# lh3/bwa

Hardware: NVIDIA H100
Metric: reads_per_sec (higher is better)
Workload: dtype int32

## Files before the change

bwa_b200/csrc/cuda/bwag_api.cu:

```cuda
#include <stdio.h>
#include <stdlib.h>
#include <string.h>
#include <stdarg.h>
#include <pthread.h>
#include <time.h>
#include <math.h>
#include <sched.h>
#include "bwag_dev.cuh"
#include "bwag_kernels.h"

struct BlobHeader {
	u64 magic, primary, seq_len, bwt_size, n_sa, l_pac;
	u64 L2[5];
	u64 sa_shift;
	u64 off_bwt, off_sa, off_pac, total;
	u64 sb[BWAG_MAX_SB][4];
};
#define BLOB_MAGIC 0x3142574142323030ull
#define ALIGN256(x) (((x) + 255) & ~(size_t)255)

static __thread char g_err[512];
extern "C" const char *bwag_last_error(void) { return g_err[0] ? g_err : "no error"; }
static int set_err(const char *fmt, ...)
{
	va_list ap;
	va_start(ap, fmt);
	vsnprintf(g_err, sizeof(g_err), fmt, ap);
	va_end(ap);
	return 1;
}
int bwag_set_error(const char *msg) { return set_err("%s", msg); }
#define CK(call) do { cudaError_t e_ = (call); if (e_ != cudaSuccess) return set_err("%s failed at %s:%d: %s", #call, __FILE__, __LINE__, cudaGetErrorString(e_)); } while (0)
#define CKP(call) do { cudaError_t e_ = (call); if (e_ != cudaSuccess) { set_err("%s failed at %s:%d: %s", #call, __FILE__, __LINE__, cudaGetErrorString(e_)); return 0; } } while (0)

struct Counters {
	int next_read, next_task, max_rlen, next_read3;
	u64 next_seed;
	u64 n_intv, n_seeds;
	u64 occ_touches, sa_touches, ext_cells, glb_cells;
	u64 n_cig, n_md;
	u32 flags, n_pre;
	u64 t_dregs, t_tasks, t_max_z, t_text, t_complex;
	int t_max_lq, t_max_rl;
	int n_many;
	int n_big;
	u32 n_swtasks;
	u64 fm_total[3];
	int aln_next;
	u32 aln_redo, aln_flags;
	u64 aln_pool, aln_total;
	u64 se_total, se_run, se_cells;
	int se_next, se_past;
	u64 pm_total;
};

struct DevBuf { void *p; size_t cap; };
static int buf_reserve(DevBuf *b, size_t bytes)
{
	if (bytes <= b->cap) return 0;
	if (b->p) cudaFree(b->p);
	b->p = 0; b->cap = 0;
	size_t want = bytes + bytes / 4 + 256;
	CK(cudaMalloc(&b->p, want));
	b->cap = want;
	return 0;
}
struct HostBuf { void *p; size_t cap; };
static int hbuf_reserve(HostBuf *b, size_t bytes)
{
	if (bytes <= b->cap) return 0;
	if (b->p) cudaFreeHost(b->p);
	b->p = 0; b->cap = 0;
	size_t want = bytes + bytes / 4 + 256;
	CK(cudaMallocHost(&b->p, want));
	b->cap = want;
	return 0;
}

struct bwag_ctx {
	int device, own_blob, n_sm;
	int imported;
	size_t map_bytes[3];
	void *blob;
	DevIndex ix;
	u64 *dense_sa;
	ulonglong2 *ktab;
	int baseline;
	cudaStream_t stream;
	cudaEvent_t ev0, ev1, ev_wait;
	Counters *d_cnt, *h_cnt;
	bwag_stats_t st;
	int sa_intv_disk;
	DevBuf s_k1, s_k1f, s_n3, s_eh, s_rseq, s_qseq, s_z, s_wcig, s_wmd, s_pack, s_zl;
	int grid_k1, grid_k1f, grid_k2, grid_k4, grid_k5;
	int k3s_blocks;
#define N_SPARE 12
	struct bwag_batch *spare[N_SPARE];
	pthread_mutex_t mu;
	struct bwag_ctx *parent;
	void *d_tail; TailCtg tctg; const double *d_logtab; int have_ctg;
	void *d_ambs; int n_holes, have_ambs;
};

struct bwag_batch {
	bwag_ctx_t *ctx;
	bwag_ctx_t lc;
	int lc_ready;
	int n;
	i64 total_bases;
	int max_len;
	const i64 *h_off;
	DevBuf d_codes, d_off;
	DevBuf d_intv_beg, d_intv_n, d_intv, d_seed_beg, d_rbeg;
	HostBuf h_intv_beg, h_intv_n, h_intv, h_seed_beg, h_rbeg;
	DevBuf d_chain_off, d_chains, d_seeds, d_regs, d_nregs;
	DevBuf d_chain_beg, d_chain_cnt, d_reg_base, d_chain_rid, d_chain_frac, d_cregs, d_creg_beg, d_ctg;
	DevBuf s_bt, s_sn, s_ch, s_order, s_idx, s_keys;
	HostBuf h_regs, h_nregs, h_cregs, h_creg_beg, h_tmp;
	i64 n_intv, n_seeds;
	int seeded;
	DevBuf d_tasks, d_res, d_cig, d_md;
	HostBuf h_res, h_cig, h_md;
	DevBuf d_dregs, d_dreg_beg, d_dreg_n, d_task_beg, d_cflag, d_pe_is, d_rec, d_text, d_ptab;
	DevBuf d_swtasks, d_swres, d_swpool, d_swscratch; HostBuf h_swres;
	DevBuf d_hsp, d_flt_nchn; HostBuf h_hsp;
	DevBuf d_k3big;
	DevBuf d_pre_n, d_pre_score, d_pre_cig;
	DevBuf d_sel;
	HostBuf h_pe_is, h_cflag, h_rec, h_text, h_ptab;
	DevBuf d_fm_lbeg, d_fm_lines, d_fm_nrow, d_fm_rbeg, d_fm_rows, d_fm_tlen, d_fm_tbeg, d_fm_text, d_fm_toff;
	HostBuf h_fm_text, h_fm_off;
	DevBuf d_aln_md, d_aln_n, d_aln_beg, d_aln_pool, d_aln_redo[2], d_aln_off, d_aln_out, d_aln_arena;
	HostBuf h_aln_n, h_aln_off, h_aln_out;
	DevBuf d_se_reads, d_se_multi, d_se_bc, d_se_rows, d_se_pos, d_se_mpos, d_se_flags, d_se_tasks, d_se_mtask, d_se_cig, d_se_ncig, d_se_scratch, d_se_tlen, d_se_tbeg, d_se_rec, d_se_text, d_se_nm;
	HostBuf h_se_tasks, h_se_mtask, h_se_rec, h_se_text;
	DevBuf d_pe_rlen, d_pe_reads, d_pe_gtasks, d_pe_gres, d_pe_gcig, d_pe_pool;
	HostBuf h_pe_pos, h_pe_gres, h_pe_gcig;
	DevBuf d_pm_qual, d_pm_hasq, d_pm_names, d_pm_noff, d_pm_q, d_pm_code, d_pm_ovl, d_pm_tlen, d_pm_tbeg, d_pm_text, d_pm_cnt;
	HostBuf h_pm_text, h_pm_cnt;
	int tail_ready;
	int regs_on_device;
};

static void batch_free(bwag_batch_t *b);
static void free_dev(DevBuf *b) { if (b->p) cudaFree(b->p); b->p = 0; b->cap = 0; }
static void free_host(HostBuf *b) { if (b->p) cudaFreeHost(b->p); b->p = 0; b->cap = 0; }

#ifndef BWAG_L2_FETCH_DEFAULT
#define BWAG_L2_FETCH_DEFAULT 0
#endif
#define K1_SMEM_MAX (200 * 1024)
#ifndef K1_COMPACT_DEFAULT
#define K1_COMPACT_DEFAULT 1
#endif
#ifdef BWAG_CUSIM
#define BWAG_KTAB_MAX_AUTO 5
#else
#define BWAG_KTAB_MAX_AUTO 14
#endif
#define K4_SMEM_MAX (96 * 1024)
#define K4L_SMEM_MAX (200 * 1024)
#define SEEDSW_MAXLEN 200

#ifdef BWAG_CUSIM
unsigned long long bwag_cusim_sector_loads, bwag_cusim_list_acc[5];
#endif


extern "C" size_t bwag_blob_bytes(const bwt_t *bwt, int64_t l_pac)
{
	return ALIGN256(sizeof(BlobHeader)) + ALIGN256((size_t)bwt->bwt_size * 4 + 64) + ALIGN256((size_t)bwt->n_sa * 8 + 32) + ALIGN256((size_t)l_pac / 4 + 1 + 64);
}

extern "C" int bwag_blob_fill(int device, void *d_blob, const bwt_t *bwt, int64_t l_pac, const uint8_t *pac)
{
	BlobHeader h;
	if (device >= 0) CK(cudaSetDevice(device));
	memset(&h, 0, sizeof(h));
	h.magic = BLOB_MAGIC; h.primary = bwt->primary; h.seq_len = bwt->seq_len; h.bwt_size = bwt->bwt_size; h.n_sa = bwt->n_sa; h.l_pac = (u64)l_pac;
	for (int i = 0; i < 5; ++i) h.L2[i] = bwt->L2[i];
	{
		int s = 0;
		while ((1 << s) < bwt->sa_intv) ++s;
		if ((1 << s) != bwt->sa_intv) return set_err("suffix-array interval %d is not a power of two", bwt->sa_intv);
		h.sa_shift = (u64)s;
	}
	if (bwt->seq_len >= (u64)BWAG_MAX_SB << BWAG_SB_SHIFT) return set_err("index too large: %llu BWT symbols", (unsigned long long)bwt->seq_len);
	for (u64 s = 0; s << BWAG_SB_SHIFT < bwt->seq_len; ++s) {
		const u64 *cnt = (const u64 *)(bwt->bwt + ((s << BWAG_SB_SHIFT) >> 7) * 16);
		for (int k = 0; k < 4; ++k) h.sb[s][k] = cnt[k];
	}
	h.off_bwt = ALIGN256(sizeof(BlobHeader));
	h.off_sa = h.off_bwt + ALIGN256((size_t)bwt->bwt_size * 4 + 64);
	h.off_pac = h.off_sa + ALIGN256((size_t)bwt->n_sa * 8 + 32);
// ... 1669 lines not shown
		CK(cudaEventRecord(c->ev0, c->stream));
		BWAG_LAUNCH(k_chain_emit, (n + K3_THREADS - 1) / K3_THREADS, K3_THREADS, 0, c->stream, k);
		CK(cudaGetLastError());
		CK(cudaEventRecord(c->ev1, c->stream));
		if (fetch_counters(c)) return 1;
		c->st.ms_chain += elapsed_at(c, "chain", __LINE__); ++c->st.n_launch;
	}

	const int cap_q = (b->max_len + 3) & ~3;
	const int cap_r = (c->h_cnt->max_rlen + 16 + 15) & ~15;
	CK(cudaMemsetAsync(&c->d_cnt->next_read, 0, sizeof(int), c->stream));
	int grid = c->grid_k4;
	{
		i64 need = ((i64)n + (K4_THREADS / 32) - 1) / (K4_THREADS / 32);
		if (grid > need) grid = (int)(need > 0 ? need : 1);
	}
	ExtArgs a;
	memset(&a, 0, sizeof(a));
	a.codes = (const uint8_t *)b->d_codes.p; a.off = (const i64 *)b->d_off.p; a.n_reads = n; a.par = *par;
	a.chain_beg = (const i64 *)b->d_chain_beg.p; a.chain_cnt = (const int *)b->d_chain_cnt.p; a.reg_base = (const i64 *)b->d_reg_base.p;
	a.chains = (const bwag_xchain_t *)b->d_chains.p; a.seeds = (const bwag_xseed_t *)b->d_seeds.p;
	a.regs = (bwag_xreg_t *)b->d_regs.p; a.n_regs = (int32_t *)b->d_nregs.p;
	a.cap_q = cap_q; a.cap_r = cap_r; a.min_seed = cp->min_seed_len;
	a.next_read = &c->d_cnt->next_read; a.cells = &c->d_cnt->ext_cells; a.flags = &c->d_cnt->flags;
	CK(cudaEventRecord(c->ev0, c->stream));
	if (launch_extend(c, a, n, c->h_cnt->n_many)) return 1;
	CK(cudaEventRecord(c->ev1, c->stream));
	if (!out) {
		if (fetch_counters(c)) return 1;
		c->st.ms_extend += elapsed_at(c, "extend", __LINE__); ++c->st.n_launch;
		if (c->h_cnt->flags & 2u) return set_err("extension: a read or reference window exceeded the scratch capacity");
		c->st.ext_cells += c->h_cnt->ext_cells;
		b->regs_on_device = 1;
		return 0;
	}
	RegCompactArgs rc;
	rc.n_reads = n; rc.n_regs = (const int *)b->d_nregs.p; rc.regs = (const bwag_xreg_t *)b->d_regs.p; rc.reg_base = (const i64 *)b->d_reg_base.p;
	rc.chain_beg = (const i64 *)b->d_chain_beg.p; rc.chain_rid = (const int *)b->d_chain_rid.p; rc.chain_frac = (const float *)b->d_chain_frac.p;
	rc.out_beg = (i64 *)b->d_creg_beg.p; rc.total = &c->d_cnt->n_cig;
	if (buf_reserve(&b->d_cregs, sizeof(bwag_creg_t) * (size_t)(ns + 1))) return 1;
	rc.out = (bwag_creg_t *)b->d_cregs.p;
	BWAG_LAUNCH(k_regs_compact, (n + 127) / 128, 128, 0, c->stream, rc);
	CK(cudaGetLastError());
	if (fetch_counters(c)) return 1;
	c->st.ms_extend += elapsed_at(c, "extend", __LINE__); c->st.n_launch += 2;
	if (c->h_cnt->flags & 2u) return set_err("extension: a read or reference window exceeded the scratch capacity");
	c->st.ext_cells += c->h_cnt->ext_cells;
	const i64 n_regs = (i64)c->h_cnt->n_cig;
	if (hbuf_reserve(&b->h_cregs, sizeof(bwag_creg_t) * (size_t)(n_regs + 1)) || hbuf_reserve(&b->h_creg_beg, 8 * (size_t)(n + 1)) || hbuf_reserve(&b->h_nregs, 4 * (size_t)(n + 1))) return 1;
	CK(cudaEventRecord(c->ev0, c->stream));
	if (n_regs) D2H(c, b->h_cregs.p, b->d_cregs.p, sizeof(bwag_creg_t) * (size_t)n_regs);
	D2H(c, b->h_creg_beg.p, b->d_creg_beg.p, 8 * (size_t)n);
	D2H(c, b->h_nregs.p, b->d_nregs.p, 4 * (size_t)n);
	CK(cudaEventRecord(c->ev1, c->stream));
	CK(stream_wait(c));
	c->st.ms_d2h += elapsed_at(c, "d2h", __LINE__);
	out->n_regs = (const int32_t *)b->h_nregs.p; out->reg_beg = (const int64_t *)b->h_creg_beg.p; out->regs = (const bwag_creg_t *)b->h_cregs.p;
	return 0;
}

extern "C" int bwag_fetch_cregs(bwag_batch_t *b, int n_sel, const int32_t *sel, bwag_cregs_t *out)
{
	bwag_ctx_t *c = &b->lc;
	CK(cudaSetDevice(c->device));
	if (!b->regs_on_device) return set_err("bwag_fetch_cregs needs a preceding bwag_chain_extend(..., NULL) on the same batch");
	out->n_regs = 0; out->reg_beg = 0; out->regs = 0;
	if (n_sel <= 0) return 0;
	const i64 ns = b->n_seeds;
	if (buf_reserve(&b->d_cregs, sizeof(bwag_creg_t) * (size_t)(ns + 1)) || buf_reserve(&b->d_creg_beg, 8 * (size_t)(b->n + 1)) || buf_reserve(&b->d_sel, 8 * (size_t)(n_sel + 1))) return 1;
	if (reset_counters(c)) return 1;
	H2D(c, b->d_sel.p, sel, 4 * (size_t)n_sel);
	RegCompactArgs rc;
	rc.n_reads = b->n; rc.n_regs = (const int *)b->d_nregs.p; rc.regs = (const bwag_xreg_t *)b->d_regs.p; rc.reg_base = (const i64 *)b->d_reg_base.p;
	rc.chain_beg = (const i64 *)b->d_chain_beg.p; rc.chain_rid = (const int *)b->d_chain_rid.p; rc.chain_frac = (const float *)b->d_chain_frac.p;
	rc.out_beg = (i64 *)b->d_creg_beg.p; rc.total = &c->d_cnt->n_cig; rc.out = (bwag_creg_t *)b->d_cregs.p;
	int *d_out_n = (int *)b->d_sel.p + n_sel;
	BWAG_LAUNCH(k_regs_compact_sel, (n_sel + 127) / 128, 128, 0, c->stream, rc, (const int *)b->d_sel.p, n_sel, d_out_n);
	CK(cudaGetLastError());
	if (fetch_counters(c)) return 1;
	++c->st.n_launch;
	const i64 n_regs = (i64)c->h_cnt->n_cig;
	if (hbuf_reserve(&b->h_cregs, sizeof(bwag_creg_t) * (size_t)(n_regs + 1)) || hbuf_reserve(&b->h_creg_beg, 8 * (size_t)(n_sel + 1)) || hbuf_reserve(&b->h_nregs, 4 * (size_t)(n_sel + 1))) return 1;
	CK(cudaEventRecord(c->ev0, c->stream));
	if (n_regs) D2H(c, b->h_cregs.p, b->d_cregs.p, sizeof(bwag_creg_t) * (size_t)n_regs);
	D2H(c, b->h_creg_beg.p, b->d_creg_beg.p, 8 * (size_t)n_sel);
	D2H(c, b->h_nregs.p, d_out_n, 4 * (size_t)n_sel);
	CK(cudaEventRecord(c->ev1, c->stream));
	CK(stream_wait(c));
	c->st.ms_d2h += elapsed_at(c, "d2h", __LINE__);
	out->n_regs = (const int32_t *)b->h_nregs.p; out->reg_beg = (const int64_t *)b->h_creg_beg.p; out->regs = (const bwag_creg_t *)b->h_cregs.p;
	return 0;
}


static int run_global(bwag_batch_t *b, const bwag_sw_par_t *par, int n_tasks, int cap_q, int cap_r, i64 cap_z, i64 n_aln, i64 *nc_out, i64 *nm_out)
{
	bwag_ctx_t *c = &b->lc;
	cap_q = (cap_q + 3) & ~3; cap_r = (cap_r + 15) & ~15; cap_z = (cap_z + 15) & ~(i64)15;
	if (cap_q < 4) cap_q = 4;
	if (cap_r < 16) cap_r = 16;
	if (cap_z < 64) cap_z = 64;
	const int cap_wcig = cap_q + cap_r + 4, cap_wmd = 3 * cap_r + cap_q + 16;
	int grid = c->grid_k5;
	const int k5_zsm = getenv("BWA_B200_K5_ZSM") ? atoi(getenv("BWA_B200_K5_ZSM")) & ~15 : 6144;
	const int k5_per_warp = ((8 * (cap_q + 2) + cap_r + cap_q + 2 + 15) & ~15) + k5_zsm;
	const size_t k5_smem = (size_t)k5_per_warp * (K5_THREADS / 32);
	int k5_sm = k5_smem <= K4_SMEM_MAX && !(getenv("BWA_B200_K5_SM") && atoi(getenv("BWA_B200_K5_SM")) == 0);
	const int k5_fast = !c->baseline && !(getenv("BWA_B200_K5_FAST") && atoi(getenv("BWA_B200_K5_FAST")) == 0);
#ifndef BWAG_CUSIM
	if (k5_sm) { int nb = 0; CK(cudaOccupancyMaxActiveBlocksPerMultiprocessor(&nb, k5_fast ? k_global_sm_fast : k_global_sm, K5_THREADS, k5_smem)); if (nb < 2) k5_sm = 0; else grid = c->n_sm * nb; }
#endif
	{
		i64 need = ((i64)n_tasks + (K5_THREADS / 32) - 1) / (K5_THREADS / 32);
		if (grid > need) grid = (int)(need > 0 ? need : 1);
		i64 max_warps = ((i64)8 << 30) / cap_z;
		if (max_warps < K5_THREADS / 32) max_warps = K5_THREADS / 32;
		if ((i64)grid * (K5_THREADS / 32) > max_warps) grid = (int)(max_warps / (K5_THREADS / 32));
	}
	const size_t n_warps = (size_t)grid * (K5_THREADS / 32);
	if (buf_reserve(&c->s_eh, n_warps * 2 * (size_t)(cap_q + 2) * 4) || buf_reserve(&c->s_rseq, n_warps * (size_t)cap_r) ||
	    buf_reserve(&c->s_qseq, n_warps * (size_t)(cap_q + 2)) || buf_reserve(&c->s_z, n_warps * (size_t)cap_z) ||
	    buf_reserve(&c->s_wcig, n_warps * (size_t)cap_wcig * 4) || buf_reserve(&c->s_wmd, n_warps * (size_t)cap_wmd)) return 1;
	if (buf_reserve(&b->d_res, sizeof(bwag_gres_t) * (size_t)n_tasks)) return 1;
	int k5_lane = !c->baseline && cap_q <= K5L_QWORDS * 4 && n_tasks >= 64 && getenv("BWA_B200_K5_LANE") && atoi(getenv("BWA_B200_K5_LANE")) != 0;
	const size_t k5l_smem = (size_t)K5L_RING * K5L_THREADS * 8 + (size_t)K5L_QWORDS * K5L_THREADS * 4;
	const i64 k5l_cap_z = (i64)(K5L_RING - 1) * (cap_r < 1024 ? cap_r : 1024);
	int k5l_grid = 0;
	if (k5_lane) {
#ifndef BWAG_CUSIM
		int nb = 0;
		CK(cudaFuncSetAttribute(k_global_lane, cudaFuncAttributeMaxDynamicSharedMemorySize, (int)k5l_smem));
		CK(cudaOccupancyMaxActiveBlocksPerMultiprocessor(&nb, k_global_lane, K5L_THREADS, k5l_smem));
		k5l_grid = c->n_sm * (nb > 0 ? nb : 1);
#else
		k5l_grid = 2;
#endif
		const i64 need = ((i64)n_tasks + K5L_THREADS - 1) / K5L_THREADS;
		if (k5l_grid > need) k5l_grid = (int)need;
		if (buf_reserve(&b->d_pre_n, 4 * (size_t)n_tasks) || buf_reserve(&b->d_pre_score, 4 * (size_t)n_tasks) || buf_reserve(&b->d_pre_cig, 4 * (size_t)K5L_MAXCIG * (size_t)n_tasks) ||
		    buf_reserve(&c->s_zl, (size_t)k5l_cap_z * (size_t)k5l_grid * K5L_THREADS)) return 1;
	}
	i64 cap_cig = n_aln * 6 + 1024, cap_md = n_aln * 24 + 4096;
	for (int attempt = 0;; ++attempt) {
		if (buf_reserve(&b->d_cig, 4 * (size_t)cap_cig) || buf_reserve(&b->d_md, (size_t)cap_md)) return 1;
		GlbArgs a;
		memset(&a, 0, sizeof(a));
		a.codes = (const uint8_t *)b->d_codes.p; a.off = (const i64 *)b->d_off.p; a.par = *par;
		a.tasks = (const bwag_gtask_t *)b->d_tasks.p; a.n_tasks = n_tasks;
		a.res = (bwag_gres_t *)b->d_res.p; a.cigar = (u32 *)b->d_cig.p; a.md = (char *)b->d_md.p;
		a.cap_cig = cap_cig; a.cap_md = cap_md; a.n_cig = &c->d_cnt->n_cig; a.n_md = &c->d_cnt->n_md;
		a.w_cig = (u32 *)c->s_wcig.p; a.w_md = (char *)c->s_wmd.p; a.cap_wcig = cap_wcig; a.cap_wmd = cap_wmd;
		a.eh = (int *)c->s_eh.p; a.rseq = (uint8_t *)c->s_rseq.p; a.qseq = (uint8_t *)c->s_qseq.p; a.z = (uint8_t *)c->s_z.p;
		a.cap_q = cap_q; a.cap_r = cap_r; a.cap_z = cap_z;
		a.next_task = &c->d_cnt->next_task; a.cells = &c->d_cnt->glb_cells; a.flags = &c->d_cnt->flags;
		if (reset_counters(c)) return 1;
		CK(cudaEventRecord(c->ev0, c->stream));
		if (k5_lane) {
			GlbLaneArgs la;
			memset(&la, 0, sizeof(la));
			la.codes = a.codes; la.off = a.off; la.par = *par; la.tasks = a.tasks; la.n_tasks = n_tasks;
			la.pre_n = (int *)b->d_pre_n.p; la.pre_score = (int *)b->d_pre_score.p; la.pre_cig = (u32 *)b->d_pre_cig.p;
			la.z = (uint8_t *)c->s_zl.p; la.cap_z = k5l_cap_z; la.next_task = &c->d_cnt->next_task; la.cells = &c->d_cnt->glb_cells; la.n_pre = &c->d_cnt->n_pre;
			BWAG_LAUNCH(k_global_lane, k5l_grid, K5L_THREADS, k5l_smem, c->stream, c->ix, la);
			CK(cudaGetLastError());
			CK(cudaMemsetAsync(&c->d_cnt->next_task, 0, sizeof(int), c->stream));
			a.pre_n = la.pre_n; a.pre_score = la.pre_score; a.pre_cig = la.pre_cig;
			++c->st.n_launch;
		}
		a.smem_per_warp = k5_sm ? k5_per_warp : 0; a.z_sm_bytes = k5_sm ? k5_zsm : 0;
		if (k5_sm && k5_fast) BWAG_LAUNCH(k_global_sm_fast, grid, K5_THREADS, k5_smem, c->stream, c->ix, a);
		else if (k5_sm) BWAG_LAUNCH(k_global_sm, grid, K5_THREADS, k5_smem, c->stream, c->ix, a);
		else if (k5_fast) BWAG_LAUNCH(k_global_fast, grid, K5_THREADS, 0, c->stream, c->ix, a);
		else BWAG_LAUNCH(k_global, grid, K5_THREADS, 0, c->stream, c->ix, a);
		CK(cudaGetLastError());
		CK(cudaEventRecord(c->ev1, c->stream));
		if (fetch_counters(c)) return 1;
		c->st.ms_global += elapsed_at(c, "global", __LINE__); ++c->st.n_launch;
		if (k5_lane && getenv("BWA_B200_PROFILE")) fprintf(stderr, "[prof] global alignment: lane-per-request kernel made %u of %d CIGARs, grid %d x %d\n", c->h_cnt->n_pre, n_tasks, k5l_grid, K5L_THREADS);
		if (c->h_cnt->flags & 4u) return set_err("global alignment: a task exceeded the scratch capacity");
		if (!(c->h_cnt->flags & 16u)) break;
		if (attempt >= 3) return set_err("global alignment: output pools keep overflowing");
		cap_cig = (i64)c->h_cnt->n_cig + 1024; cap_md = (i64)c->h_cnt->n_md + 4096;
	}
	c->st.glb_cells += c->h_cnt->glb_cells;
	*nc_out = (i64)c->h_cnt->n_cig; *nm_out = (i64)c->h_cnt->n_md;
	return 0;
}

extern "C" int bwag_global(bwag_batch_t *b, const bwag_sw_par_t *par, int n_tasks, const bwag_gtask_t *tasks, bwag_galn_t *out)
{
	bwag_ctx_t *c = &b->lc;
	CK(cudaSetDevice(c->device));
	if (n_tasks <= 0) { out->res = 0; out->cigar = 0; out->md = 0; return 0; }
	i64 cap_z = 64, n_aln = 0, nc = 0, nm = 0;
	int cap_q = 4, cap_r = 16;
	for (int t = 0; t < n_tasks; ++t) {
		i64 lq = tasks[t].qe - tasks[t].qb, rl = tasks[t].re - tasks[t].rb;
		if (lq > cap_q) cap_q = (int)lq;
		if (rl > cap_r) cap_r = (int)rl;
		if (tasks[t].mode == BWAG_G_REG2ALN) {
			i64 d = rl > lq ? rl - lq : lq - rl, wmax = (i64)par->w << 2;
			if (d + 3 > wmax) wmax = d + 3;
			i64 ncol = lq < 2 * wmax + 1 ? lq : 2 * wmax + 1;
			if (ncol * rl > cap_z) cap_z = ncol * rl;
			++n_aln;
		}
	}
	if (buf_reserve(&b->d_tasks, sizeof(bwag_gtask_t) * (size_t)n_tasks)) return 1;
	CK(cudaEventRecord(c->ev0, c->stream));
	H2D(c, b->d_tasks.p, tasks, sizeof(bwag_gtask_t) * (size_t)n_tasks);
	CK(cudaEventRecord(c->ev1, c->stream));
	CK(stream_wait(c));
	c->st.ms_h2d += elapsed_at(c, "h2d", __LINE__);
	b->tail_ready = 0;
	if (run_global(b, par, n_tasks, cap_q, cap_r, cap_z, n_aln, &nc, &nm)) return 1;
	if (hbuf_reserve(&b->h_res, sizeof(bwag_gres_t) * (size_t)n_tasks) || hbuf_reserve(&b->h_cig, 4 * (size_t)(nc + 1)) || hbuf_reserve(&b->h_md, (size_t)nm + 16)) return 1;
	CK(cudaEventRecord(c->ev0, c->stream));
	D2H(c, b->h_res.p, b->d_res.p, sizeof(bwag_gres_t) * (size_t)n_tasks);
	if (nc) D2H(c, b->h_cig.p, b->d_cig.p, 4 * (size_t)nc);
	if (nm) D2H(c, b->h_md.p, b->d_md.p, (size_t)nm);
	CK(cudaEventRecord(c->ev1, c->stream));
	CK(stream_wait(c));
	c->st.ms_d2h += elapsed_at(c, "d2h", __LINE__);
	out->res = (const bwag_gres_t *)b->h_res.p; out->cigar = (const uint32_t *)b->h_cig.p; out->md = (const char *)b->h_md.p;
	return 0;
}


#define TAIL_LOGN 4096
extern "C" int bwag_ctx_set_contigs(bwag_ctx_t *c, int n_seqs, const int64_t *offset, const int32_t *len, const uint8_t *is_alt, const char *const *names)
{
	CK(cudaSetDevice(c->device));
	size_t l_names = 0;
	for (int i = 0; i < n_seqs; ++i) l_names += strlen(names[i]);
	const size_t o_off = 0, o_log = o_off + 8 * (size_t)n_seqs, o_len = o_log + 8 * TAIL_LOGN, o_noff = o_len + 4 * (size_t)n_seqs, o_alt = o_noff + 4 * ((size_t)n_seqs + 1), o_names = o_alt + (size_t)n_seqs, total = o_names + l_names + 16;
	char *h = (char *)malloc(total);
	if (!h) return set_err("out of memory");
	memset(h, 0, total);
	memcpy(h + o_off, offset, 8 * (size_t)n_seqs);
	memcpy(h + o_len, len, 4 * (size_t)n_seqs);
	memcpy(h + o_alt, is_alt, (size_t)n_seqs);
	{
		int *no = (int *)(h + o_noff), at = 0;
		for (int i = 0; i < n_seqs; ++i) { const size_t l = strlen(names[i]); no[i] = at; memcpy(h + o_names + at, names[i], l); at += (int)l; }
		no[n_seqs] = at;
		double *lt = (double *)(h + o_log);
		for (int i = 0; i < TAIL_LOGN; ++i) lt[i] = log((double)i);
	}
	pthread_mutex_lock(&c->mu);
	if (c->d_tail) { cudaStreamSynchronize(c->stream); cudaFree(c->d_tail); c->d_tail = 0; c->have_ctg = 0; }
	cudaError_t e = cudaMalloc(&c->d_tail, total);
	if (e == cudaSuccess) e = cudaMemcpy(c->d_tail, h, total, cudaMemcpyHostToDevice);
	free(h);
	if (e != cudaSuccess) { pthread_mutex_unlock(&c->mu); return set_err("contig table upload failed: %s", cudaGetErrorString(e)); }
	char *d = (char *)c->d_tail;
	c->tctg.l_pac = c->ix.l_pac; c->tctg.n_seqs = n_seqs;
	c->tctg.off = (const i64 *)(d + o_off); c->tctg.len = (const int *)(d + o_len); c->tctg.alt = (const uint8_t *)(d + o_alt);
	c->tctg.names = d + o_names; c->tctg.name_off = (const int *)(d + o_noff);
	c->d_logtab = (const double *)(d + o_log);
	c->have_ctg = 1;
	pthread_mutex_unlock(&c->mu);
	return 0;
}

extern "C" int bwag_tail_regs(bwag_batch_t *b, const mem_opt_t *opt, const bwag_sw_par_t *sp, const uint64_t **pe_is, const uint8_t **cflag)
{
	bwag_ctx_t *c = &b->lc, *pc = b->ctx;
	CK(cudaSetDevice(c->device));
	if (!pc->have_ctg) return BWAG_UNSUPPORTED;
	if (c->baseline) return BWAG_DECLINED;
	if (!b->regs_on_device) return set_err("bwag_tail_regs needs a preceding bwag_chain_extend(..., NULL) on the same batch");
	const int n = b->n, pe = !!(opt->flag & MEM_F_PE);
	if (pe && (n & 1)) return set_err("paired-end batch with an odd number of reads");
	const i64 cap = b->n_seeds + 1;
	if (buf_reserve(&b->d_dregs, sizeof(mem_alnreg_t) * (size_t)cap) || buf_reserve(&b->d_tasks, sizeof(bwag_gtask_t) * (size_t)cap) ||
	    buf_reserve(&b->d_dreg_beg, 8 * (size_t)(n + 1)) || buf_reserve(&b->d_dreg_n, 4 * (size_t)(n + 1)) || buf_reserve(&b->d_task_beg, 8 * (size_t)(n + 1)) ||
	    buf_reserve(&b->d_cflag, (size_t)n + 16) || buf_reserve(&b->d_pe_is, 8 * (size_t)(n / 2 + 1))) return 1;
	TailRegsArgs a;
	memset(&a, 0, sizeof(a));
	a.n_reads = n; a.pe = pe; a.opt = *opt; a.ctg = pc->tctg;
	a.n_raw = (const int *)b->d_nregs.p; a.xregs = (const bwag_xreg_t *)b->d_regs.p; a.reg_base = (const i64 *)b->d_reg_base.p; a.chain_beg = (const i64 *)b->d_chain_beg.p;
	a.chain_rid = (const int *)b->d_chain_rid.p; a.chain_frac = (const float *)b->d_chain_frac.p;
	a.dregs = (mem_alnreg_t *)b->d_dregs.p; a.dreg_beg = (i64 *)b->d_dreg_beg.p; a.dreg_n = (int *)b->d_dreg_n.p; a.task_beg = (i64 *)b->d_task_beg.p; a.cflag = (uint8_t *)b->d_cflag.p;
	a.cap_dregs = cap; a.tasks = (bwag_gtask_t *)b->d_tasks.p; a.cap_tasks = cap; a.pe_is = (u64 *)b->d_pe_is.p;
	a.n_dregs = &c->d_cnt->t_dregs; a.n_tasks = &c->d_cnt->t_tasks; a.max_z = &c->d_cnt->t_max_z; a.max_lq = &c->d_cnt->t_max_lq; a.max_rl = &c->d_cnt->t_max_rl;
	if (reset_counters(c)) return 1;
	const int n_units = pe ? n >> 1 : n;
	CK(cudaEventRecord(c->ev0, c->stream));
	BWAG_LAUNCH(k_tail_regs, (n_units + 127) / 128, 128, 0, c->stream, a);
	CK(cudaGetLastError());
	CK(cudaEventRecord(c->ev1, c->stream));
	if (fetch_counters(c)) return 1;
	c->st.ms_tail += elapsed_at(c, "tail", __LINE__); ++c->st.n_launch;
	const i64 n_tasks = (i64)c->h_cnt->t_tasks;
	if (n_tasks > cap || (i64)c->h_cnt->t_dregs > cap) return set_err("stage 4: more regions than seeds?");
	if (n_tasks >= ((i64)1 << 31)) return set_err("stage 4: too many alignment requests in one batch; use smaller chunks");
	const int cap_q = c->h_cnt->t_max_lq, cap_r = c->h_cnt->t_max_rl;
	const i64 cap_z = (i64)c->h_cnt->t_max_z;
	if (n_tasks > 0) {
		i64 nc = 0, nm = 0;
		if (run_global(b, sp, (int)n_tasks, cap_q, cap_r, cap_z, n_tasks, &nc, &nm)) return 1;
	}
	if (hbuf_reserve(&b->h_cflag, (size_t)n + 16) || hbuf_reserve(&b->h_pe_is, 8 * (size_t)(n / 2 + 1))) return 1;
	CK(cudaEventRecord(c->ev0, c->stream));
	D2H(c, b->h_cflag.p, b->d_cflag.p, (size_t)n);
	if (pe) D2H(c, b->h_pe_is.p, b->d_pe_is.p, 8 * (size_t)(n / 2));
	CK(cudaEventRecord(c->ev1, c->stream));
	CK(stream_wait(c));
	c->st.ms_d2h += elapsed_at(c, "d2h", __LINE__);
	b->tail_ready = 1;
	if (pe_is) *pe_is = pe ? (const uint64_t *)b->h_pe_is.p : 0;
	if (cflag) *cflag = (const uint8_t *)b->h_cflag.p;
	return 0;
}

extern "C" int bwag_tail_sam(bwag_batch_t *b, const mem_opt_t *opt, const mem_pestat_t pes[4], const double *const pair_tab[4], const double *log_tab,
                             int64_t n_processed, const char *rg_id, bwag_sam_t *out)
{
	bwag_ctx_t *c = &b->lc, *pc = b->ctx;
	(void)log_tab;
	CK(cudaSetDevice(c->device));
	if (!pc->have_ctg) return BWAG_UNSUPPORTED;
	if (!b->tail_ready) return set_err("bwag_tail_sam needs a preceding bwag_tail_regs on the same batch");
	const int n = b->n, pe = !!(opt->flag & MEM_F_PE);
	TailSamArgs g;
	memset(&g, 0, sizeof(g));
	g.n_reads = n; g.pe = pe; g.opt = *opt; g.ctg = pc->tctg; g.logtab = pc->d_logtab; g.n_processed = n_processed;
	size_t tab_bytes = 256;
	if (pe) {
		memcpy(g.pes, pes, 4 * sizeof(mem_pestat_t));
		for (int d = 0; d < 4; ++d) if (pair_tab && pair_tab[d] && !pes[d].failed && pes[d].high >= pes[d].low) tab_bytes += 8 * ((size_t)pes[d].high - pes[d].low + 1);
	}
	if (buf_reserve(&b->d_ptab, tab_bytes) || hbuf_reserve(&b->h_ptab, tab_bytes)) return 1;
	{
		char *h = (char *)b->h_ptab.p;
		size_t at = 256;
		const size_t l_rg = rg_id ? strlen(rg_id) : 0;
// ... 50 lines not shown
```

bwa_b200/csrc/cuda/bwag_global.cu:

```cuda
#include "bwag_dev.cuh"
#include "bwag_kernels.h"
#include "bwag_ksw.cuh"

template <class A, class AM>
__device__ __forceinline__ int warp_ksw_global_fast(int lane, int qlen, typename A::addr qa, int tlen, typename A::addr ta, typename AM::addr ma,
                               int o_del, int e_del, int o_ins, int e_ins, int w, typename A::addr he, uint8_t *z, int n_col, u64 *cells)
{
	const int oe_del = o_del + e_del, oe_ins = o_ins + e_ins;
	for (int j = lane; j <= qlen; j += 32) A::st_he(he + 8 * j, j == 0 ? 0 : (j <= w ? -(o_ins + e_ins * j) : NEG_INF), NEG_INF);
	__syncwarp();
	const bool lane0 = lane == 0;
	const int le = lane * e_ins;
	for (int i = 0; i < tlen; ++i) {
		const typename AM::addr srow = ma + A::ld_u8(ta + i) * 5;
		const int beg = i > w ? i - w : 0, end = i + w + 1 < qlen ? i + w + 1 : qlen;
		int carry_h = beg == 0 ? -(o_del + e_del * (i + 1)) : NEG_INF;
		int carry_f = NEG_INF;
		uint8_t *zi = z ? z + (i64)i * n_col - beg : 0;
		if (end > beg) *cells += (u64)(end - beg);
		for (int j0 = beg; j0 < end; j0 += 32) {
			const int j = j0 + lane;
			const bool act = j < end;
			const int jc = act ? j : end - 1;
			const int2 c = A::ld_he(he + 8 * jc);
			const int m = c.x + AM::ld_s8(srow + A::ld_u8(qa + jc));
			const int tt = act ? m - oe_ins : -0x7f000000;
			int s = tt;
			if (lane0) s = __viaddmax_s32(carry_f, -e_ins, s);
			s += le;
			{ const int v = __shfl_up_sync(FULL_MASK, s, 1); s = s > v ? s : v; }
			{ const int v = __shfl_up_sync(FULL_MASK, s, 2); s = s > v ? s : v; }
			{ const int v = __shfl_up_sync(FULL_MASK, s, 4); s = s > v ? s : v; }
			{ const int v = __shfl_up_sync(FULL_MASK, s, 8); s = s > v ? s : v; }
			{ const int v = __shfl_up_sync(FULL_MASK, s, 16); s = s > v ? s : v; }
			int f = __shfl_up_sync(FULL_MASK, s, 1) - le + e_ins;
			if (lane0) f = carry_f;
			carry_f = __shfl_sync(FULL_MASK, s, 31) - 31 * e_ins;
			int d = m >= c.y ? 0 : 1, h = m >= c.y ? m : c.y;
			d = h >= f ? d : 2; h = h >= f ? h : f;
			if (!act) h = NEG_INF;
			int hp = __shfl_up_sync(FULL_MASK, h, 1);
			if (lane0) hp = carry_h;
			{
				int la = end - 1 - j0; la = la < 31 ? la : 31;
				carry_h = __shfl_sync(FULL_MASK, h, la);
			}
			const int te = m - oe_del, ed = c.y - e_del;
			d |= ed > te ? 1 << 2 : 0;
			d |= (f - e_ins) > tt ? 2 << 4 : 0;
			if (act) {
				A::st_he(he + 8 * j, hp, ed > te ? ed : te);
				if (zi) zi[j] = (uint8_t)d;
			}
		}
		if (lane0) A::st_he(he + 8 * end, carry_h, NEG_INF);
		__syncwarp();
	}
	return A::ld_he(he + 8 * qlen).x;
}

__device__ __forceinline__ int md_put_num(char *md, int l, int v)
{
	char buf[12];
	int n = 0;
	do { buf[n++] = (char)('0' + v % 10); v /= 10; } while (v);
	while (n) md[l++] = buf[--n];
	return l;
}

template <bool C, class X, class Y> struct SelG { typedef X type; };
template <class X, class Y> struct SelG<false, X, Y> { typedef Y type; };

template <bool SM, bool FAST>
__device__ __forceinline__ void global_body(const DevIndex &ix, const GlbArgs &a)
{
	const int lane = threadIdx.x & 31;
	const i64 wid = ((i64)blockIdx.x * blockDim.x + threadIdx.x) >> 5;
	int *H, *E;
	uint8_t *rseq, *qseq, *z_glob = a.z + wid * a.cap_z, *z_sm = 0;
	if (SM) {
#ifdef BWAG_CUSIM
		unsigned char *dyn = cusim_dyn_smem;
#else
		extern __shared__ int4 k5_dyn[];
		unsigned char *dyn = reinterpret_cast<unsigned char *>(k5_dyn);
#endif
		unsigned char *mine = dyn + (size_t)(threadIdx.x >> 5) * a.smem_per_warp;
		H = reinterpret_cast<int *>(mine); E = H + a.cap_q + 2;
		rseq = reinterpret_cast<uint8_t *>(E + a.cap_q + 2);
		qseq = rseq + a.cap_r;
		if (a.z_sm_bytes) z_sm = mine + a.smem_per_warp - a.z_sm_bytes;
	} else {
		H = a.eh + wid * (i64)(2 * (a.cap_q + 2)); E = H + a.cap_q + 2;
		rseq = a.rseq + wid * (i64)a.cap_r; qseq = a.qseq + wid * (i64)(a.cap_q + 2);
	}
	typedef typename SelG<SM, SmemAcc, PtrAcc>::type A;
	typename A::addr he_a = A::make(H), rs_a = A::make(rseq), q_a = A::make(qseq);
	if constexpr (SM && FAST) { BWAG_KEEP(he_a); BWAG_KEEP(rs_a); BWAG_KEEP(q_a); }
	const bwag_sw_par_t &p = a.par;
	__shared__ int8_t s_mat[32];
	if (threadIdx.x < 25) s_mat[threadIdx.x] = p.mat[threadIdx.x];
	__syncthreads();
	typename SmemAcc::addr mat_a = SmemAcc::make(s_mat);
	if constexpr (FAST) BWAG_KEEP(mat_a);
	u64 cells = 0;
	int overflow = 0;

	for (;;) {
		int tix = 0;
		if (lane == 0) tix = atomicAdd(a.next_task, 1);
		tix = __shfl_sync(FULL_MASK, tix, 0);
		if (tix >= a.n_tasks) break;
		const bwag_gtask_t tk = a.tasks[tix];
		const int lq = tk.qe - tk.qb;
		const i64 rb = tk.rb, re = tk.re;
		u32 *cig = a.w_cig + wid * (i64)a.cap_wcig;
		char *md = a.w_md + wid * (i64)a.cap_wmd;
		int score = 0, n_cigar = 0, NM = -1, l_md = 0;
		bool ok = !(lq <= 0 || rb >= re || (rb < ix.l_pac && re > ix.l_pac)) && rb >= 0 && re <= ix.l_pac << 1;
		const int rlen = (int)(re - rb);
		if (ok && (lq > a.cap_q || rlen > a.cap_r)) { ok = false; overflow |= 4; }
		if (ok) {
			const uint8_t *query = a.codes + a.off[tk.read] + tk.qb;
			const bool rev = rb >= ix.l_pac;
			__syncwarp();
			for (int x = lane; x < rlen; x += 32) rseq[rev ? rlen - 1 - x : x] = (uint8_t)bwag_ref_base(ix, rb + x);
			for (int x = lane; x < lq; x += 32) qseq[rev ? lq - 1 - x : x] = query[x];
			__syncwarp();
			const int want = tk.mode == BWAG_G_REG2ALN;
			int w2 = tk.w, it = 0, last_sc = -(1 << 30);
			const bool have_pre = a.pre_n && a.pre_n[tix] >= 0;
			for (;;) {
				if (want) w2 = w2 < p.w << 2 ? w2 : p.w << 2;
				n_cigar = 0;
				if (have_pre) {
					score = a.pre_score[tix]; n_cigar = a.pre_n[tix];
					for (int x = lane; x < n_cigar; x += 32) cig[x] = a.pre_cig[(i64)tix * K5L_MAXCIG + x];
					__syncwarp();
				} else if (lq == rlen && w2 == 0) {
					int sc = 0;
					for (int x = lane; x < lq; x += 32) sc += s_mat[rseq[x] * 5 + qseq[x]];
					score = __reduce_add_sync(FULL_MASK, sc);
					if (want) { cig[0] = (u32)lq << 4; n_cigar = 1; }
				} else {
					int w, max_gap, max_ins, max_del, min_w, d = rlen - lq;
					d = d < 0 ? -d : d;
					max_ins = (int)((double)(((lq + 1) >> 1) * s_mat[0] - p.o_ins) / p.e_ins + 1.);
					max_del = (int)((double)(((lq + 1) >> 1) * s_mat[0] - p.o_del) / p.e_del + 1.);
					max_gap = max_ins > max_del ? max_ins : max_del;
					max_gap = max_gap > 1 ? max_gap : 1;
					w = (max_gap + d + 1) >> 1;
					w = w < w2 ? w : w2;
					min_w = d + 3;
					w = w > min_w ? w : min_w;
					const int n_col = lq < 2 * w + 1 ? lq : 2 * w + 1;
					if (want && (i64)n_col * rlen > a.cap_z) { overflow |= 4; score = 0; break; }
					uint8_t *z = z_sm && (i64)n_col * rlen <= a.z_sm_bytes ? z_sm : z_glob;
					if constexpr (FAST) score = warp_ksw_global_fast<A, SmemAcc>(lane, lq, q_a, rlen, rs_a, mat_a, p.o_del, p.e_del, p.o_ins, p.e_ins, w, he_a, want ? z : 0, n_col, &cells);
					else score = warp_ksw_global(lane, lq, qseq, rlen, rseq, s_mat, p.o_del, p.e_del, p.o_ins, p.e_ins, w, H, E, want ? z : 0, n_col, &cells);
					if (want) {
						if (lane == 0) n_cigar = ksw_backtrack(z, n_col, rlen, lq, w, cig);
						n_cigar = __shfl_sync(FULL_MASK, n_cigar, 0);
						__syncwarp();
					}
				}
				if (want) {
					const char *b2c = rev ? "TGCAN" : "ACGTN";
					int x = 0, y = 0, u = 0, n_mm = 0, n_gap = 0;
					l_md = 0;
					for (int k = 0; k < n_cigar; ++k) {
						const int op = cig[k] & 0xf, len = (int)(cig[k] >> 4);
						if (op == 0) {
							for (int b0 = 0; b0 < len; b0 += 32) {
								const int b = b0 + lane;
								const bool mm = b < len && qseq[x + b] != rseq[y + b];
								u32 bal = __ballot_sync(FULL_MASK, mm);
								n_mm += __popc(bal);
								if (lane == 0) {
									int done = 0;
									while (bal) {
										int pos = __ffs(bal) - 1;
										u += pos - done;
										l_md = md_put_num(md, l_md, u);
										md[l_md++] = b2c[rseq[y + b0 + pos]];
										u = 0; done = pos + 1;
										bal &= bal - 1;
									}
									int blk = len - b0 < 32 ? len - b0 : 32;
									u += blk - done;
								}
							}
							x += len; y += len;
						} else if (op == 2) {
							if (k > 0 && k < n_cigar - 1) {
								if (lane == 0) {
									l_md = md_put_num(md, l_md, u);
									md[l_md++] = '^';
									for (int b = 0; b < len; ++b) md[l_md++] = b2c[rseq[y + b]];
									u = 0;
								}
								n_gap += len;
							}
							y += len;
						} else if (op == 1) { x += len; n_gap += len; }
					}
					if (lane == 0) { l_md = md_put_num(md, l_md, u); md[l_md++] = 0; }
					l_md = __shfl_sync(FULL_MASK, l_md, 0);
					NM = n_mm + n_gap;
				}
				if (!want || have_pre) break;
				if (score == last_sc || w2 == p.w << 2) break;
				last_sc = score;
				w2 <<= 1;
				if (!(++it < 3 && score < tk.truesc - p.a)) break;
			}
		}
		i64 co = 0, mo = 0;
		if (n_cigar || l_md) {
			if (lane == 0) { co = (i64)atomicAdd(a.n_cig, (u64)n_cigar); mo = (i64)atomicAdd(a.n_md, (u64)((l_md + 3) & ~3)); }
			co = __shfl_sync(FULL_MASK, co, 0); mo = __shfl_sync(FULL_MASK, mo, 0);
			__syncwarp();
			if (co + n_cigar <= a.cap_cig && mo + l_md <= a.cap_md) {
				for (int x = lane; x < n_cigar; x += 32) a.cigar[co + x] = cig[x];
				for (int x = lane; x < l_md; x += 32) a.md[mo + x] = md[x];
			} else overflow |= 16;
			__syncwarp();
		}
		if (lane == 0) {
			bwag_gres_t r;
			r.score = score; r.n_cigar = n_cigar; r.NM = NM; r.l_md = l_md; r.cigar_off = co; r.md_off = mo;
			a.res[tix] = r;
		}
	}
	if (lane == 0 && cells) atomicAdd(a.cells, cells);
	if (overflow && lane == 0) atomicOr(a.flags, (u32)overflow);
}

#ifndef K5_MINB
#define K5_MINB 6
#endif
__global__ void __launch_bounds__(K5_THREADS) k_global(DevIndex ix, GlbArgs a) { global_body<false, false>(ix, a); }
__global__ void __launch_bounds__(K5_THREADS) k_global_sm(DevIndex ix, GlbArgs a) { global_body<true, false>(ix, a); }
__global__ void __launch_bounds__(K5_THREADS, K5_MINB) k_global_fast(DevIndex ix, GlbArgs a) { global_body<false, true>(ix, a); }
__global__ void __launch_bounds__(K5_THREADS, K5_MINB) k_global_sm_fast(DevIndex ix, GlbArgs a) { global_body<true, true>(ix, a); }
```

bwa_b200/csrc/cuda/bwag_kernels.h:

```cpp
#ifndef BWAG_KERNELS_H
#define BWAG_KERNELS_H
#include "bwag_dev.cuh"

#define K1_THREADS 128
#define K1F_THREADS 128
#ifndef K1_SLOTS
#ifdef K1_PACKED8
#define K1_SLOTS 8
#else
#define K1_SLOTS 4
#endif
#endif
#define K1C_SLOTS 8
#define K1B_THREADS 128
#define K2_THREADS 128
#define K3_THREADS 128
#ifndef K3S_CAP
#define K3S_CAP 16
#endif
#define K3S_THREADS 64
#define K3S_SMEM (K3S_THREADS * (62 * K3S_CAP + 21 * (1 + (K3S_CAP - 1) / 4) + 4))
#define K4_THREADS 128
#define K5_THREADS 128
#define K4L_THREADS 128
#ifndef K4L_MINB
#define K4L_MINB 3
#endif

struct Intv;

int bwag_set_error(const char *msg);

struct SeedArgs {
	const uint8_t *codes; const i64 *off; int n_reads;
	int min_seed_len, split_len, split_width, max_occ; u64 max_mem_intv;
	Intv *scratch; int cap_list, cap_mem;
	int qstride;
	int pstride;
	int nstride;
	Intv *stage3; int cap3; int *n3; int *next_read3;
	int post_copies3;
	const u32 *packed;
	const u32 *nmask;
	const u32 *hasn;
	i64 *intv_beg; int *intv_n; bwtintv_t *intv; i64 *seed_beg; i64 *rbeg;
	i64 cap_intv, cap_seeds;
	int *next_read; u64 *n_intv; u64 *n_seeds; u64 *occ_touches; u32 *flags;
};

struct SaArgs { i64 *rbeg; i64 n; u64 *next; u64 *sa_touches; };

struct ChainArgs {
	const i64 *off; int n_reads;
	const i64 *intv_beg; const int *intv_n; const bwtintv_t *intv; const i64 *seed_beg; const i64 *rbeg;
	int w, max_chain_gap, max_occ, min_seed_len, min_chain_weight, max_chain_extend; float mask_level, drop_ratio;
	int a, o_del, e_del, o_ins, e_ins;
	i64 l_pac; int n_seqs; const i64 *ctg_off; const int *ctg_len; const uint8_t *ctg_alt;
	void *s_bt, *s_sn, *s_ch; int *s_order, *s_idx; u64 *s_keys;
	bwag_xchain_t *xchains; bwag_xseed_t *xseeds; int *chain_rid; float *chain_frac;
	i64 *chain_beg, *reg_base; int *n_chains;
	int *max_rlen;
	int *n_many; int many;
	const int *hsp_tab; bwag_swtask_t *sw_tasks; u32 *n_swtasks; const bwag_swres_t *sw_res; int *flt_nchn;
	int *big; int *n_big;
	u32 *k3clk;
};

struct RegCompactArgs {
	int n_reads; const int *n_regs; const bwag_xreg_t *regs; const i64 *reg_base, *chain_beg; const int *chain_rid; const float *chain_frac;
	i64 *out_beg; bwag_creg_t *out; u64 *total;
};

struct ExtArgs {
	const uint8_t *codes; const i64 *off; int n_reads;
	bwag_sw_par_t par;
	const i64 *chain_beg; const int *chain_cnt; const i64 *reg_base;
	const bwag_xchain_t *chains; const bwag_xseed_t *seeds;
	bwag_xreg_t *regs; int32_t *n_regs;
	int *eh; uint8_t *rseq; int cap_q, cap_r;
	int smem_per_warp;
	int min_seed;
	int chain_lo, chain_hi;
	int *next_read; u64 *cells; u32 *flags;
};

struct GlbArgs {
	const uint8_t *codes; const i64 *off;
	bwag_sw_par_t par;
	const bwag_gtask_t *tasks; int n_tasks;
	bwag_gres_t *res; u32 *cigar; char *md;
	i64 cap_cig, cap_md; u64 *n_cig, *n_md;
	u32 *w_cig; char *w_md; int cap_wcig, cap_wmd;
	int *eh; uint8_t *rseq; uint8_t *qseq; uint8_t *z;
	int cap_q, cap_r; i64 cap_z;
	int smem_per_warp;
	int z_sm_bytes;
	int *next_task; u64 *cells; u32 *flags;
	const int *pre_n, *pre_score; const u32 *pre_cig;
};

#define K5L_THREADS 128
#define K5L_RING 64
#define K5L_QWORDS 64
#define K5L_MAXCIG 16
struct GlbLaneArgs {
	const uint8_t *codes; const i64 *off;
	bwag_sw_par_t par;
	const bwag_gtask_t *tasks; int n_tasks;
	int *pre_n, *pre_score; u32 *pre_cig;
	uint8_t *z; i64 cap_z;
	int *next_task; u64 *cells; u32 *n_pre;
};

struct TailCtg { i64 l_pac; int n_seqs; const i64 *off; const int *len; const uint8_t *alt; const char *names; const int *name_off; };
__device__ __forceinline__ int t_pos2rid(const TailCtg &c, i64 pos_f)
{
	int lo = 0, hi = c.n_seqs, mid = 0;
	if (pos_f >= c.l_pac) return -1;
	while (lo < hi) {
		mid = (lo + hi) >> 1;
		if (pos_f < c.off[mid]) hi = mid;
		else if (mid == c.n_seqs - 1 || pos_f < c.off[mid + 1]) break;
		else lo = mid + 1;
	}
	return mid;
}

struct TailRegsArgs {
	int n_reads, pe;
	mem_opt_t opt;
	TailCtg ctg;
	const int *n_raw; const bwag_xreg_t *xregs; const i64 *reg_base, *chain_beg; const int *chain_rid; const float *chain_frac;
	mem_alnreg_t *dregs; i64 *dreg_beg; int *dreg_n; i64 *task_beg; uint8_t *cflag; i64 cap_dregs;
	bwag_gtask_t *tasks; i64 cap_tasks;
	u64 *pe_is;
	u64 *n_dregs, *n_tasks, *max_z; int *max_lq, *max_rl;
};

struct TailSamArgs {
	int n_reads, pe;
	mem_opt_t opt;
	TailCtg ctg;
	mem_pestat_t pes[4];
	const double *ptab[4];
	const double *logtab;
	i64 n_processed;
	const uint8_t *codes; const i64 *off;
	const mem_alnreg_t *dregs; const i64 *dreg_beg; const int *dreg_n; const i64 *task_beg; const uint8_t *cflag;
	const bwag_gres_t *res; const u32 *cigar; const char *md;
	const char *rg; int l_rg;
	bwag_samrec_t *rec; char *text; i64 cap_text; u64 *n_text, *n_complex;
};

struct SwArgs {
	const bwag_swtask_t *tasks; int n_tasks;
	bwag_sw_par_t par;
	const uint8_t *codes;
	const uint8_t *pool;
	bwag_swres_t *res;
	unsigned char *scratch; i64 per_thread; int cap_n, cap_q, cap_t;
	int *next_task; u32 *flags;
};

#define FM_SCAN_THREADS 1024
struct FmArgs {
	int n_reads; i64 n_lines;
	u64 max_iwidth;
	TailCtg ctg;
	const i64 *intv_beg; const int *intv_n; const bwtintv_t *intv;
	const i64 *lbeg;
	bwtintv_t *lines; i64 *nrow;
	const i64 *rbeg; i64 *rows;
	i64 *tlen; const i64 *tbeg; char *text;
	i64 *toff;
};
__global__ void k_fm_scan32(const int *in, i64 n, i64 *out, u64 *total);
__global__ void k_fm_scan64(const i64 *in, i64 n, i64 *out, u64 *total);
__global__ void k_fm_lines(FmArgs a);
__global__ void k_fm_rows(FmArgs a);
__global__ void k_fm_text(FmArgs a, int write);
__global__ void k_fm_readoff(FmArgs a);
__global__ void k_smem_fm(DevIndex ix, SeedArgs a, int min_intv, u64 max_intv);

#define ALN_THREADS 128
struct AlnNode { u64 k, l; u32 pos, cnt, id; int next; };
struct AlnLayout { i64 heads, mask, ww, wb, sw, sb, nodes, bytes; };
__host__ __device__ __forceinline__ AlnLayout aln_layout(int n_buckets, int max_len, int seed_cap, i64 cap_nodes)
{
	AlnLayout L;
	i64 o = 0;
	L.heads = o; o += (4 * (i64)n_buckets + 15) & ~(i64)15;
	L.mask = o;  o += (8 * (i64)((n_buckets + 63) / 64) + 15) & ~(i64)15;
	L.ww = o;    o += (8 * (i64)(max_len + 1) + 15) & ~(i64)15;
	L.wb = o;    o += (4 * (i64)(max_len + 1) + 15) & ~(i64)15;
	L.sw = o;    o += (8 * (i64)(seed_cap + 1) + 15) & ~(i64)15;
	L.sb = o;    o += (4 * (i64)(seed_cap + 1) + 15) & ~(i64)15;
	L.nodes = o; o += (i64)sizeof(AlnNode) * cap_nodes;
	L.bytes = o;
	return L;
}
struct AlnArgs {
	const uint8_t *codes; const i64 *off;
	bwag_aln_par_t par;
	int n_buckets;
	const int *work; int n_work;
	unsigned char *arena; i64 lane_bytes;
	int cap_nodes, max_len, seed_cap, n_lanes;
	int *n_aln; i64 *hit_beg;
	bwag_aln1_t *pool; i64 cap_pool; u64 *n_pool;
	int *redo; u32 *n_redo; u32 *flags;
	int *next;
};
__global__ void k_aln(DevIndex ix, AlnArgs a);
__global__ void k_aln_gather(int n_reads, const int *n_aln, const i64 *hit_beg, const bwag_aln1_t *pool, const i64 *off, bwag_aln1_t *out);

#define SE_THREADS 128
struct SeTask { int read, slot; i64 cig_off; };
struct SeArgs {
	int n_reads; i64 n_multi; int n_tasks;
	int mode, max_top2; const char *rg; int l_rg;
	TailCtg ctg; int n_holes; const i64 *amb_off; const int *amb_len;
	const uint8_t *codes; const i64 *off;
	const bwag_se_read_t *reads; const bwag_se_hit_t *multi; const char *bc;
	i64 *rows;
	i64 *pos; uint8_t *strand, *mapped;
	i64 *mpos; uint8_t *mstrand, *mkeep;
	const SeTask *tasks; const int *main_task, *multi_task;
	u32 *cig; int *ncig; int *tshift;
	int *eh; uint8_t *rseq, *qseq, *z; int cap_q, cap_r; i64 cap_z;
	int *next_task; int *past_end; u64 *n_run, *cells;
	i64 *tlen; const i64 *tbeg; char *text; bwag_samrec_t *rec;
	int *nm;
};
__global__ void k_se_rows(SeArgs a);
__global__ void k_se_pos(SeArgs a);
__global__ void k_se_refine(DevIndex ix, SeArgs a);
__global__ void k_se_text(DevIndex ix, SeArgs a, int write);

struct PePosArgs { i64 n, l_pac; const i64 *rows; const int *ref_len; i64 *pos; uint8_t *strand; };
struct PeGlbArgs {
	int n_tasks; const bwag_pe_gtask_t *tasks; bwag_pe_gres_t *res; u32 *cig; const uint8_t *pool;
	int *eh; uint8_t *rseq, *z; int cap_q, cap_r; i64 cap_z;
	int *next_task; u64 *cells;
};
__global__ void k_pe_pos(PePosArgs a);
__global__ void k_pe_global(DevIndex ix, PeGlbArgs a);
__global__ void k_pe_text(DevIndex ix, SeArgs a, const bwag_pe_read_t *pe, int write);

struct PemArgs {
	int n_pairs, T, q_thres, q_def, flag;
	const uint8_t *raw; const i64 *off;
// ... 46 lines not shown
```

Baseline: 13.45 million.

## Add anti-diagonal wavefront warp kernel for narrow-band global alignment

```diff
diff --git a/bwa_b200/csrc/cuda/bwag_api.cu b/bwa_b200/csrc/cuda/bwag_api.cu
--- a/bwa_b200/csrc/cuda/bwag_api.cu
+++ b/bwa_b200/csrc/cuda/bwag_api.cu
@@ -40,6 +40,7 @@
 	u64 occ_touches, sa_touches, ext_cells, glb_cells;
 	u64 n_cig, n_md;
 	u32 flags, n_pre;
+	u32 glb_mix[3];
 	u64 t_dregs, t_tasks, t_max_z, t_text, t_complex;
 	int t_max_lq, t_max_rl;
 	int n_many;
@@ -2015,7 +2016,7 @@
 		a.w_cig = (u32 *)c->s_wcig.p; a.w_md = (char *)c->s_wmd.p; a.cap_wcig = cap_wcig; a.cap_wmd = cap_wmd;
 		a.eh = (int *)c->s_eh.p; a.rseq = (uint8_t *)c->s_rseq.p; a.qseq = (uint8_t *)c->s_qseq.p; a.z = (uint8_t *)c->s_z.p;
 		a.cap_q = cap_q; a.cap_r = cap_r; a.cap_z = cap_z;
-		a.next_task = &c->d_cnt->next_task; a.cells = &c->d_cnt->glb_cells; a.flags = &c->d_cnt->flags;
+		a.next_task = &c->d_cnt->next_task; a.cells = &c->d_cnt->glb_cells; a.flags = &c->d_cnt->flags; a.mix = c->d_cnt->glb_mix;
 		if (reset_counters(c)) return 1;
 		CK(cudaEventRecord(c->ev0, c->stream));
 		if (k5_lane) {
@@ -2046,6 +2047,9 @@
 		cap_cig = (i64)c->h_cnt->n_cig + 1024; cap_md = (i64)c->h_cnt->n_md + 4096;
 	}
 	c->st.glb_cells += c->h_cnt->glb_cells;
+	if (getenv("BWA_B200_PROFILE"))
+		fprintf(stderr, "[prof] global: %d requests, %u gap-free, %u wave sweeps, %u row sweeps, %llu cells\n", n_tasks, c->h_cnt->glb_mix[0],
+		        c->h_cnt->glb_mix[1], c->h_cnt->glb_mix[2], (unsigned long long)c->h_cnt->glb_cells);
 	*nc_out = (i64)c->h_cnt->n_cig; *nm_out = (i64)c->h_cnt->n_md;
 	return 0;
 }
diff --git a/bwa_b200/csrc/cuda/bwag_global.cu b/bwa_b200/csrc/cuda/bwag_global.cu
--- a/bwa_b200/csrc/cuda/bwag_global.cu
+++ b/bwa_b200/csrc/cuda/bwag_global.cu
@@ -59,6 +59,65 @@
 	return A::ld_he(he + 8 * qlen).x;
 }
 
+#define K5_WAVE_K 8
+#define K5_WAVE_WMAX ((63 - K5_WAVE_K) / 2)
+template <class A, class AM, class Z>
+__device__ __forceinline__ int warp_ksw_global_wave(int lane, int qlen, typename A::addr qa, int tlen, typename A::addr ta, typename AM::addr ma,
+                               int o_del, int e_del, int o_ins, int e_ins, int w, typename Z::addr z, bool rec, int n_col, u64 *cells)
+{
+	const int oe_del = o_del + e_del, oe_ins = o_ins + e_ins, src = (lane + 31) & 31;
+	int i = lane - 32, beg = 0, c = 0, width = 0, h1 = NEG_INF, f = NEG_INF, out_h = 0, out_e = NEG_INF, ncell = 0;
+	typename A::addr qrow = qa;
+	typename AM::addr srow = ma;
+	typename Z::addr zrow = z;
+	auto next_row = [&](int a1) {
+		i += 32;
+		beg = i > w ? i - w : 0;
+		const int end = i + w + 1 < qlen ? i + w + 1 : qlen;
+		if (i < tlen && end > beg) {
+			width = end - beg; ncell += width;
+			c = a1 - (i + beg);
+			h1 = beg == 0 ? -(o_del + e_del * (i + 1)) : NEG_INF; f = NEG_INF;
+			qrow = qa + beg; srow = ma + A::ld_u8(ta + i) * 5; zrow = z + i * n_col;
+		} else { width = 0; c = -(1 << 30); qrow = qa; srow = ma; }
+	};
+	next_row(0);
+	auto step = [&](int a, bool first) {
+		if (first && lane == 31) { out_h = a == 0 ? 0 : -(o_ins + e_ins * a); out_e = NEG_INF; }
+		const int dh = __shfl_sync(FULL_MASK, out_h, src), e = __shfl_sync(FULL_MASK, out_e, src);
+		const bool act = (unsigned)c < (unsigned)width;
+		const int m = dh + AM::ld_s8(srow + A::ld_u8(qrow + (act ? c : 0)));
+		int d = m >= e ? 0 : 1, h = m >= e ? m : e;
+		d = h >= f ? d : 2; h = h >= f ? h : f;
+		const int te = m - oe_del, ed = e - e_del, tf = m - oe_ins, fd = f - e_ins;
+		d |= ed > te ? 1 << 2 : 0;
+		d |= fd > tf ? 2 << 4 : 0;
+		out_h = h1;
+		out_e = act ? (ed > te ? ed : te) : NEG_INF;
+		h1 = act ? h : h1;
+		f = act ? (fd > tf ? fd : tf) : f;
+		if (act && rec) Z::st_u8(zrow + c, d);
+		++c;
+	};
+	const int il = tlen - 1 < qlen + w - 1 ? tlen - 1 : qlen + w - 1;
+	const int a_last = il + (il + w + 1 < qlen ? il + w + 1 : qlen) - 1;
+	const int end0 = w + 1 < qlen ? w + 1 : qlen;
+	int a = 0;
+	for (; a < end0; a += K5_WAVE_K) {
+#pragma unroll
+		for (int k = 0; k < K5_WAVE_K; ++k) step(a + k, true);
+		if (c > width && width > 0) next_row(a + K5_WAVE_K);
+	}
+	for (; a <= a_last; a += K5_WAVE_K) {
+#pragma unroll
+		for (int k = 0; k < K5_WAVE_K; ++k) step(a + k, false);
+		if (c > width && width > 0) next_row(a + K5_WAVE_K);
+	}
+	*cells += (u64)(u32)__reduce_add_sync(FULL_MASK, ncell);
+	const int hl = __shfl_sync(FULL_MASK, h1, (tlen - 1) & 31);
+	return tlen - 1 == il && il + w + 1 >= qlen ? hl : NEG_INF;
+}
+
 __device__ __forceinline__ int md_put_num(char *md, int l, int v)
 {
 	char buf[12];
@@ -104,6 +163,7 @@
 	typename SmemAcc::addr mat_a = SmemAcc::make(s_mat);
 	if constexpr (FAST) BWAG_KEEP(mat_a);
 	u64 cells = 0;
+	u32 n_free = 0, n_wave = 0, n_rows = 0;
 	int overflow = 0;
 
 	for (;;) {
@@ -138,6 +198,7 @@
 					for (int x = lane; x < n_cigar; x += 32) cig[x] = a.pre_cig[(i64)tix * K5L_MAXCIG + x];
 					__syncwarp();
 				} else if (lq == rlen && w2 == 0) {
+					if (it == 0) ++n_free;
 					int sc = 0;
 					for (int x = lane; x < lq; x += 32) sc += s_mat[rseq[x] * 5 + qseq[x]];
 					score = __reduce_add_sync(FULL_MASK, sc);
@@ -156,8 +217,19 @@
 					const int n_col = lq < 2 * w + 1 ? lq : 2 * w + 1;
 					if (want && (i64)n_col * rlen > a.cap_z) { overflow |= 4; score = 0; break; }
 					uint8_t *z = z_sm && (i64)n_col * rlen <= a.z_sm_bytes ? z_sm : z_glob;
-					if constexpr (FAST) score = warp_ksw_global_fast<A, SmemAcc>(lane, lq, q_a, rlen, rs_a, mat_a, p.o_del, p.e_del, p.o_ins, p.e_ins, w, he_a, want ? z : 0, n_col, &cells);
-					else score = warp_ksw_global(lane, lq, qseq, rlen, rseq, s_mat, p.o_del, p.e_del, p.o_ins, p.e_ins, w, H, E, want ? z : 0, n_col, &cells);
+					if constexpr (FAST) {
+						if (w <= K5_WAVE_WMAX) {
+							++n_wave;
+							if (SM && z == z_sm) score = warp_ksw_global_wave<A, SmemAcc, SmemAcc>(lane, lq, q_a, rlen, rs_a, mat_a, p.o_del, p.e_del, p.o_ins, p.e_ins, w, SmemAcc::make(z), want, n_col, &cells);
+							else score = warp_ksw_global_wave<A, SmemAcc, PtrAcc>(lane, lq, q_a, rlen, rs_a, mat_a, p.o_del, p.e_del, p.o_ins, p.e_ins, w, PtrAcc::make(z), want, n_col, &cells);
+						} else {
+							++n_rows;
+							score = warp_ksw_global_fast<A, SmemAcc>(lane, lq, q_a, rlen, rs_a, mat_a, p.o_del, p.e_del, p.o_ins, p.e_ins, w, he_a, want ? z : 0, n_col, &cells);
+						}
+					} else {
+						++n_rows;
+						score = warp_ksw_global(lane, lq, qseq, rlen, rseq, s_mat, p.o_del, p.e_del, p.o_ins, p.e_ins, w, H, E, want ? z : 0, n_col, &cells);
+					}
 					if (want) {
 						if (lane == 0) n_cigar = ksw_backtrack(z, n_col, rlen, lq, w, cig);
 						n_cigar = __shfl_sync(FULL_MASK, n_cigar, 0);
@@ -233,6 +305,9 @@
 		}
 	}
 	if (lane == 0 && cells) atomicAdd(a.cells, cells);
+	if (lane == 0 && n_free) atomicAdd(a.mix + 0, n_free);
+	if (lane == 0 && n_wave) atomicAdd(a.mix + 1, n_wave);
+	if (lane == 0 && n_rows) atomicAdd(a.mix + 2, n_rows);
 	if (overflow && lane == 0) atomicOr(a.flags, (u32)overflow);
 }
 
diff --git a/bwa_b200/csrc/cuda/bwag_kernels.h b/bwa_b200/csrc/cuda/bwag_kernels.h
--- a/bwa_b200/csrc/cuda/bwag_kernels.h
+++ b/bwa_b200/csrc/cuda/bwag_kernels.h
@@ -97,6 +97,7 @@
 	int z_sm_bytes;
 	int *next_task; u64 *cells; u32 *flags;
 	const int *pre_n, *pre_score; const u32 *pre_cig;
+	u32 *mix;
 };
 
 #define K5L_THREADS 128
```

New measurement: 13.91 million (median of 6 runs). +3.4%, better.
